# spool-labs/tape

Hardware: AMD Instinct MI355X
Metric: device-resident encode GiB/s, batched 4 MiB objects, 1 MI355X; % HBM peak (higher is better)
Workload: dtype u8; 1 GPU; Slicer::encode of 1024 x 4194304 B objects per GPU, Clay(20,7,16) rotated, 1 MB stripes; objects_per_gpu=1024, object_bytes=4194304, parallelism=objects partitioned over 1 GPU(s)

## Files before the change

### tape_amd/csrc/encode_dma.hip

```cpp
#include <atomic>
#include <string.h>
#include "kernels.hpp"
#include "gf_dev.hpp"
#include "dev_io.hpp"
#include "enc_common.hpp"

namespace tec {
namespace dma {

using enc::kQ;
using enc::pft3;
constexpr int K = 7;
constexpr int G = 6;
constexpr uint32_t RB = 90;
constexpr uint32_t RW = RB * 16;
constexpr uint32_t kOwnBlk = 7 * RB;
constexpr uint32_t kPartBlk = 9 * RB;
constexpr uint32_t kPartBase = kOwnBlk * 16;
constexpr uint32_t kSlotBytes = (kOwnBlk + kPartBlk) * 16;
constexpr uint32_t kRing = 2;
constexpr uint32_t kStageBase = kRing * kSlotBytes;
constexpr uint32_t kStageRows = 24;
constexpr uint32_t kMailBase = kStageBase + kStageRows * RW;
constexpr uint32_t kMailBytes = 64;
// ... 341 lines not shown
#if TEC_DMA_JX
        const uint32_t jx_base = (uint32_t)(reinterpret_cast<uintptr_t>(jdst) & 127u);
        const __amdgpu_buffer_rsrc_t rb_jx =
            __builtin_amdgcn_make_buffer_rsrc(jdst - jx_base, 0, (int)(dst_range + jx_base), 0x00020000);
#endif
        const uint32_t store_mask = J.store_mask;
        uint32_t sl_lane = lane + J.rot;
        sl_lane = (sl_lane >= 20u ? sl_lane - 20u : sl_lane) * slen;
        auto slice_off = [&](uint32_t node) -> uint32_t { return __builtin_amdgcn_readlane(sl_lane, node); };

        for (uint32_t z0 = z0b; z0 < z0e; z0++) {
            const bool lvl2 = z0 >= (uint32_t)K;
            const uint32_t type = lvl2 ? z0 - (K - 1) : 0u;
            for (uint32_t s = 0; s < (uint32_t)kQ; s++) {
                const uint32_t z = z0 * kQ + s;
                const uint32_t slot = (z & 1u) * kSlotBytes;
                const uint8_t *img = lds8 + slot + colw;
                auto out = [&](int r, uint32_t v) { st32(stg + r * RW, v); };
                uint32_t own[K], part[kQ];
#pragma unroll
                for (int x = 0; x < K; x++) own[x] = lds32(img + x * RW);
                if (z == ez && fixl) {
#pragma unroll
                    for (int x = 0; x < K; x++)
                        if ((uint32_t)x == ex) own[x] = fixw;
                    st32(lds8 + slot + ex * RW + colw, fixw);
                }
                uint32_t acc[20 - K];
                if (!lvl2) {
#pragma unroll
                    for (int x = 0; x < kQ; x++)
                        part[x] = lds32(img + kPartBase + x * RW - ((uint32_t)x > z0 ? RW : 0u));
                    if (z0 == ex && s == ez % kQ && fixl) {
#pragma unroll
                        for (int x = 0; x < kQ; x++)
                            if ((uint32_t)x == ez / kQ) part[x] = fixw;
                    }
                    uint32_t u[K];
#pragma unroll
                    for (int x = 0; x < K; x++) u[x] = (uint32_t)x == z0 ? own[x] : pft3(own[x], part[x]);
                    enc::mds7_slp<true>(u, acc);
#pragma unroll
                    for (int r = 0; r < 3; r++)
                        out(kRowC0 + r, acc[r] ^ mulc(kPft.t_p[1], part[K + r]));
                } else {
#pragma unroll
                    for (int x = 0; x < 9; x++) part[x] = lds32(img + kPartBase + x * RW);
                    uint32_t u[K];
#pragma unroll
                    for (int x = 0; x < K; x++) u[x] = pft3(own[x], part[x]);
                    enc::mds7_slp<false>(u, acc);
                    const uint32_t i0 = z0 - K;
#pragma unroll
                    for (int r = 0; r < 3; r++) {
                        if (r < 2) {
                            const uint32_t us = part[K + r], up = acc[r];
                            const uint32_t tt = xt(us ^ up);
                            out(kRowX + r, us ^ tt);
                            out(kRowC0 + r, (uint32_t)r < i0 ? up ^ tt : up);
                        } else {
                            out(kRowC0 + r, acc[r]);
                        }
                    }
                }
                switch (s) {
                    case 0: col1<0>(acc + 3, sl, out); break;
                    case 1: col1<1>(acc + 3, sl, out); break;
                    case 2: col1<2>(acc + 3, sl, out); break;
                    case 3: col1<3>(acc + 3, sl, out); break;
                    case 4: col1<4>(acc + 3, sl, out); break;
                    case 5: col1<5>(acc + 3, sl, out); break;
                    case 6: col1<6>(acc + 3, sl, out); break;
                    case 7: col1<7>(acc + 3, sl, out); break;
                    case 8: col1<8>(acc + 3, sl, out); break;
                    default: col1<9>(acc + 3, sl, out); break;
                }
                lds_barrier();
                const FlushTab::W &F = kFlush.w[type][s][wv];
                const uint32_t n = F.n;
                u32x4 d0[kCap], d1[kCap];
                uint32_t dst[kCap];
#pragma unroll
                for (int q = 0; q < kCap; q++) {
                    if ((uint32_t)q < n) {
                        const uint32_t it = F.item[q];
                        const uint32_t src = it & 0xffu;
                        const uint8_t *row = (src & 0x80u) ? lds8 + slot + (src & 0x7fu) * RW : lds8 + kStageBase + src * RW;
                        d0[q] = *reinterpret_cast<const u32x4 *>(row + lo0);
                        d1[q] = *reinterpret_cast<const u32x4 *>(row + lo1);
                        const uint32_t node = (it >> 8) & 0xffu, tz0 = (it >> 16) & 0xffu, ts = it >> 24;
                        dst[q] = slice_off(node) + ((tz0 == 0xffu ? z0 : tz0) * kQ + (ts == 0xffu ? s : ts)) * sc;
                        if (!((store_mask >> node) & 1u)) dst[q] = kDrop;
                    }
                }
                asm volatile("s_waitcnt vmcnt(%0)" ::"n"(kStoreLag) : "memory");
                lds_barrier();
#pragma unroll
                for (int q = 0; q < kCap; q++) {
                    if ((uint32_t)q < n) {
#if TEC_DMA_JX
                        const uint32_t ab = jx_base + dst[q], first = (ab + 127u) & ~127u;
                        const uint32_t o0 = first + 16u * lane - jx_base, o1 = first + 16u * (64u + lane) - jx_base;
                        const uint32_t lim = ((ab + (uint32_t)sc + 127u) & ~127u) - jx_base;
                        __builtin_amdgcn_raw_buffer_store_b128(d0[q], rb_jx, (int)(dst[q] == kDrop ? kDrop : o0), 0, kStAux);
                        __builtin_amdgcn_raw_buffer_store_b128(d1[q], rb_jx, (int)(dst[q] == kDrop || o1 >= lim ? kDrop : o1), 0, kStAux);
#else
                        __builtin_amdgcn_raw_buffer_store_b128(d0[q], rb_dst, (int)vo0, (int)dst[q], kStAux);
                        __builtin_amdgcn_raw_buffer_store_b128(d1[q], rb_dst, (int)vo1, (int)dst[q], kStAux);
#endif
                    }
                }
            }
        }
        if (wv == 0 && z0e == (uint32_t)kQ) {
            const uint32_t it = kFlush.extra, src = it & 0xffu;
            const uint8_t *row = lds8 + kStageBase + src * RW;
            const u32x4 e0 = *reinterpret_cast<const u32x4 *>(row + lo0);
            const u32x4 e1 = *reinterpret_cast<const u32x4 *>(row + lo1);
            const uint32_t node = (it >> 8) & 0xffu, tz0 = (it >> 16) & 0xffu, ts = it >> 24;
            const uint32_t d = ((store_mask >> node) & 1u)
                                   ? slice_off(node) + ((tz0 == 0xffu ? kQ - 1u : tz0) * kQ + (ts == 0xffu ? kQ - 1u : ts)) * sc
                                   : kDrop;
            __builtin_amdgcn_raw_buffer_store_b128(e0, rb_dst, (int)vo0, (int)d, kStAux);
            __builtin_amdgcn_raw_buffer_store_b128(e1, rb_dst, (int)vo1, (int)d, kStAux);
        }
    }
}

}

bool encode_dma_supported(int n, int k, uint32_t sc) { return n == 20 && k == 7 && sc > 1280u && sc <= 1440u && sc % 2 == 0; }

static uint32_t enc_slots() {
    const char *e = tec_knob("TEC_ENC_GRID");
    if (e && strcmp(e, "cu") != 0) {
        const long v = atol(e);
        return v < 0 ? 0u : (uint32_t)v;
    }
    static std::atomic<uint32_t> cached[64];
    int dev = 0;
    if (hipGetDevice(&dev) != hipSuccess || dev < 0 || dev >= 64) dev = 0;
    uint32_t v = cached[dev].load(std::memory_order_relaxed);
    if (!v) {
        int cus = 0;
        if (hipDeviceGetAttribute(&cus, hipDeviceAttributeMultiprocessorCount, dev) != hipSuccess || cus <= 0) cus = 256;
        v = 2u * (uint32_t)cus;
        cached[dev].store(v, std::memory_order_relaxed);
    }
    return v;
}

uint32_t encode_dma_grid(const EncArgs &a) { return enc_grid(enc_task_count(a), enc_slots()); }

hipError_t launch_encode_dma(bool masked, const EncArgs &a0, hipStream_t s) {
    if (a0.njobs == 0) return hipSuccess;
    if (!encode_dma_supported((int)a0.n, 7, a0.sc) || a0.njobs > 0x7fffffffu) return hipErrorInvalidValue;
    const void *fn = masked ? reinterpret_cast<const void *>(dma::enc_dma_kernel<true>)
                            : reinterpret_cast<const void *>(dma::enc_dma_kernel<false>);
#ifndef TEC_DMA_LDS_PAD
#define TEC_DMA_LDS_PAD 0
#endif
    const size_t lds = dma::kLdsBytes + TEC_DMA_LDS_PAD;
    hipError_t e = ensure_dyn_lds(fn, lds);
    if (e != hipSuccess) return e;
    if (a0.z0_count) {
        const uint32_t lim = a0.z0_limit ? a0.z0_limit : 10u;
        if (a0.z0_split == 0 || lim > 10u || a0.z0_first + (a0.z0_split - 1u) * a0.z0_count >= lim) return hipErrorInvalidValue;
    }
    const uint64_t ntasks = enc_task_count(a0);
    if (ntasks > 0x7fffffffu) return hipErrorInvalidValue;
    EncArgs a = a0;
    a.ntasks = (uint32_t)ntasks;
    const uint32_t grid = a.queue ? encode_dma_grid(a) : a.ntasks;
    if (masked)
        hipLaunchKernelGGL(dma::enc_dma_kernel<true>, dim3(grid), dim3(dma::kWaves * 64), lds, s, a);
    else
        hipLaunchKernelGGL(dma::enc_dma_kernel<false>, dim3(grid), dim3(dma::kWaves * 64), lds, s, a);
    return hipGetLastError();
}

}
```

### tape_amd/csrc/engine.cpp

```cpp
#include <hip/hip_runtime.h>
#include <string.h>
#include <stdio.h>
#include <stdlib.h>
#include <deque>
#include <map>
#include <unordered_map>
#include <mutex>
#include <vector>
#include <algorithm>
#include <functional>
#include <thread>
#include <atomic>
#include <chrono>
#include <condition_variable>
#include "../../include/tape_ec.h"
#include "kernels.hpp"
#include "sha256.hpp"
#include <array>
#include "clay_host.hpp"
#include "rs16.hpp"
#include "host_hash.hpp"
#include "copy_pool.hpp"
#include "dec_class.hpp"

using namespace tec;

namespace {

constexpr size_t kStripeSizes[3] = {100000, 1000000, 10000000};

thread_local char g_last_error[256] = "";
const bool g_no_dma_encode = [] {
    const char *e = tec_knob("TEC_ENCODE_KERNEL");
    return e && strcmp(e, "stage") == 0;
}();

const uint32_t g_enc_split = [] {
    const char *e = tec_knob("TEC_ENC_SPLIT");
    return e ? (uint32_t)atoi(e) : 512u;
}();
const uint32_t g_enc_split_batch = [] {
    const char *e = tec_knob("TEC_ENC_SPLIT_BATCH");
    const int v = e ? atoi(e) : 0;
    return (uint32_t)(v < 0 ? 0 : v > 7 ? 7 : v);
}();
const uint32_t g_enc_small = [] {
    const char *e = tec_knob("TEC_ENC_SMALL");
    return e ? (uint32_t)atoi(e) : 0u;
}();

const bool g_no_fold_repair = [] {
    const char *e = tec_knob("TEC_REPAIR_KERNEL");
    return e && strcmp(e, "stage") == 0;
}();

int hip_status(hipError_t e) {
    if (e == hipSuccess) return TE_OK;
    snprintf(g_last_error, sizeof(g_last_error), "%s (%d)", hipGetErrorString(e), (int)e);
    if (e == hipErrorOutOfMemory) return TE_ERR_OUT_OF_MEMORY;
    if (e == hipErrorNoDevice || e == hipErrorInvalidDevice) return TE_ERR_NO_DEVICE;
    return TE_ERR_HIP;
}

#define TE_HIP(expr)                              \
    do {                                          \
        hipError_t e_ = (expr);                   \
        if (e_ != hipSuccess) return hip_status(e_); \
    } while (0)

int sync_sleep(hipStream_t s) {
    hipEvent_t e = nullptr;
    if (hipEventCreateWithFlags(&e, hipEventDisableTiming | hipEventBlockingSync) != hipSuccess)
        return hip_status(hipStreamSynchronize(s));
    hipError_t r = hipEventRecord(e, s);
    if (r == hipSuccess) r = hipEventSynchronize(e);
    (void)hipEventDestroy(e);
    return hip_status(r);
}

int g_device_count = -1;
std::mutex g_dev_mu;

int device_count() {
    std::lock_guard<std::mutex> lk(g_dev_mu);
    if (g_device_count < 0) {
        int n = 0;
        if (hipGetDeviceCount(&n) != hipSuccess) n = 0;
        g_device_count = n;
    }
    return g_device_count;
}

struct DeviceGuard {
    int prev = -1;
    hipError_t err = hipSuccess;
    explicit DeviceGuard(int dev) {
        if (hipGetDevice(&prev) != hipSuccess) prev = -1;
        if (prev != dev) err = hipSetDevice(dev);
    }
    ~DeviceGuard() {
        int cur = -1;
        if (prev >= 0 && hipGetDevice(&cur) == hipSuccess && cur != prev) (void)hipSetDevice(prev);
    }
};

static bool vmm_bufs() {
    static const bool v = [] {
        const char *s = tec_knob("TEC_VMM_BUFS");
        return s && s[0] == '1';
    }();
    return v;
}

struct ReaderEvents {
    struct E {
        hipStream_t s = nullptr;
        hipEvent_t ev = nullptr;
        bool pending = false;
    };
    static constexpr size_t kMax = 16;
    std::vector<E> v;
    bool any() const {
        for (const E &e : v)
            if (e.pending) return true;
        return false;
    }
    hipError_t record(hipStream_t s) {
        E *slot = nullptr;
        for (E &e : v)
            if (e.s == s) slot = &e;
        if (!slot) {
            if (v.size() >= kMax) {
                if (hipError_t r = sync(); r != hipSuccess) return r;
                slot = &v[0];
                slot->s = s;
            } else {
                E e;
                e.s = s;
                if (hipError_t r = hipEventCreateWithFlags(&e.ev, hipEventDisableTiming); r != hipSuccess) return r;
                v.push_back(e);
                slot = &v.back();
            }
        }
        hipError_t r = hipEventRecord(slot->ev, s);
        if (r == hipSuccess) slot->pending = true;
        return r;
    }
    hipError_t wait(hipStream_t s) const {
        for (const E &e : v)
            if (e.pending && e.s != s)
                if (hipError_t r = hipStreamWaitEvent(s, e.ev, 0); r != hipSuccess) return r;
        return hipSuccess;
    }
    hipError_t sync() {
        for (E &e : v)
            if (e.pending) {
                if (hipError_t r = hipEventSynchronize(e.ev); r != hipSuccess) return r;
                e.pending = false;
            }
        return hipSuccess;
    }
    void destroy() {
        for (E &e : v)
            if (e.ev) (void)hipEventDestroy(e.ev);
        v.clear();
    }
};

static tec::CopyPool &copy_pool(int device) {
    static std::mutex mu;
    static tec::CopyPool *pools[65] = {};
    const int slot = device < 0 || device >= 64 ? 64 : device;
    std::lock_guard<std::mutex> g(mu);
    if (!pools[slot]) pools[slot] = new tec::CopyPool(std::max(0, std::min(3, hh::default_threads() - 1)));
    return *pools[slot];
}

struct DevBuf {
    void *p = nullptr;
    size_t cap = 0;
    hipMemGenericAllocationHandle_t vh{};
    bool vmm = false;
    hipError_t free_() {
        if (!p) return hipSuccess;
        hipError_t e = hipSuccess;
        if (vmm) {
            (void)hipDeviceSynchronize();
            e = hipMemUnmap(p, cap);
            if (e == hipSuccess) e = hipMemRelease(vh);
            if (e == hipSuccess) e = hipMemAddressFree(p, cap);
        } else {
            e = hipFree(p);
        }
        p = nullptr;
        cap = 0;
        vmm = false;
        return e;
    }
// ... 572 lines not shown
int te_slice_metadata_from_slice(const uint8_t *slice, size_t len, te_slice_metadata *out) {
    if (!slice || !out || len < TE_META_SIZE) return TE_ERR_INVALID_LAYOUT;
    const uint8_t *p = slice + len - TE_META_SIZE;
    out->version = get_u64(p);
    out->blob_len = get_u64(p + 8);
    out->stripe_size = get_u64(p + 16);
    out->encoding = get_u64(p + 24);
    out->params = get_u64(p + 32);
    out->chunk_index = get_u64(p + 40);
    if (!valid_stripe(out->stripe_size)) return TE_ERR_INVALID_LAYOUT;
    return TE_OK;
}

int te_slicer_geometry(const te_clay *c, size_t blob_len, te_geometry *g) {
    if (!c || !g) return TE_ERR_INVALID_ARG;
    const size_t S = te_pick_stripe_size(blob_len);
    const size_t ns = te_num_stripes(blob_len, S);
    const size_t eff = blob_len == 0 ? S : std::min(blob_len, S);
    const size_t cs = c->h.chunk_size_for(eff);
    g->stripe_size = S;
    g->num_stripes = ns;
    g->chunk_size = cs;
    g->sub_chunk_size = cs / (size_t)c->h.alpha;
    g->slice_len = ns * cs + TE_META_SIZE;
    return TE_OK;
}

}

namespace {

struct GeomKey {
    uint64_t cs, slice_len;
    bool masked;
    bool odd;
    bool operator<(const GeomKey &o) const {
        if (cs != o.cs) return cs < o.cs;
        if (slice_len != o.slice_len) return slice_len < o.slice_len;
        if (odd != o.odd) return odd < o.odd;
        return masked < o.masked;
    }
};

int ensure_stream(te_clay *c) {
    if (device_count() <= 0) return TE_ERR_NO_DEVICE;
    if (!c->stream) TE_HIP(hipStreamCreateWithFlags(&c->stream, hipStreamNonBlocking));
    return TE_OK;
}

using StripeSel = std::function<uint32_t(size_t, size_t)>;

int encode_enqueue(te_clay *c, const te_slicer_cfg *cfg, const uint8_t *d_data, const te_object *objs,
                   size_t nobj, uint8_t *d_out, hipStream_t s, bool raw, Arena *arena = nullptr,
                   const StripeSel &keep = StripeSel(), bool per_call = false) {
    const ClayHost &h = c->h;
    const int n = h.n;
    const int rotated = cfg ? cfg->rotated : 0;
    std::map<GeomKey, std::vector<EncJob>> groups;
    std::vector<MetaJob> metas;

    for (size_t i = 0; i < nobj; i++) {
        const te_object &o = objs[i];
        size_t S, ns, cs, slice_len;
        if (raw) {
            if (o.blob_len == 0) return TE_ERR_EMPTY_INPUT;
            cs = h.chunk_size_for(o.blob_len);
            S = cs * h.k;
            ns = 1;
            slice_len = cs;
        } else {
            te_geometry g;
            te_slicer_geometry(c, o.blob_len, &g);
            S = g.stripe_size; ns = g.num_stripes; cs = g.chunk_size; slice_len = g.slice_len;
        }
        if (cs % (size_t)h.alpha || slice_len > 0xffffffffull || cs > 0xffffffffull) return TE_ERR_TOO_MUCH_DATA;
        for (size_t st = 0; st < ns; st++) {
            const uint32_t store = keep ? keep(i, st) : ~0u;
            if (!store) continue;
            EncJob j{};
            j.store_mask = store;
            const uint64_t start = (uint64_t)st * S;
            j.src = d_data + o.data_off + start;
            j.src_len = o.blob_len == 0 ? 0 : std::min<uint64_t>(S, o.blob_len - start);
            j.dst = d_out + o.out_off + st * cs;
            j.rot = rotated ? (uint32_t)((st * TE_ROTATION_STEP) % n) : 0u;
            j.dst_skew = (uint32_t)(st * cs);
            const bool masked = ((reinterpret_cast<uintptr_t>(j.src) & 3u) + j.src_len) % 4 != 0;
            const bool odd = (reinterpret_cast<uintptr_t>(j.src) & 1u) != 0;
            groups[GeomKey{cs, slice_len, masked, odd}].push_back(j);
        }
        if (!raw && !keep) {
            MetaJob m{};
            m.dst = d_out + o.out_off + ns * cs;
            m.slice_len = slice_len;
            m.words[0] = 0;
            m.words[1] = o.blob_len;
            m.words[2] = S;
            m.words[3] = cfg ? cfg->encoding : TE_ENCODING_CLAY;
            m.words[4] = cfg ? cfg->params : TE_CLAY_DEFAULT_PARAMS;
            m.words[5] = o.chunk_index;
            metas.push_back(m);
        }
    }
    Arena &A = arena ? *arena : c->enc;
    A.img.clear();
    struct Launch { GeomKey key; size_t off, count; };
    std::vector<Launch> launches;
    for (auto &kv : groups) launches.push_back({kv.first, A.put(kv.second.data(), kv.second.size() * sizeof(EncJob)), kv.second.size()});
    const size_t meta_off = A.put(metas.data(), metas.size() * sizeof(MetaJob));
    size_t pat_off = 0, pool_off = 0;
    GpePattern pat{};
    std::vector<uint16_t> pool;
    std::vector<GpeJob> gjobs;
    std::vector<size_t> gjob_off;
    {
        uint64_t mask = 0;
        for (int i = h.k + h.nu; i < h.qt; i++) mask |= 1ull << i;
        if (!h.gpe_pattern(mask, pat, pool)) return TE_ERR_UNSUPPORTED;
        pat_off = A.put(&pat, sizeof(pat));
        pool_off = A.put(pool.data(), pool.size() * sizeof(uint16_t));
        for (auto &kv : groups) {
            std::vector<GpeJob> gj;
            for (const EncJob &e : kv.second) {
                GpeJob g{};
                g.in = e.src; g.out = e.dst; g.in_len = e.src_len; g.out_len = ~0ull; g.rot = e.rot; g.pattern = 0;
                gj.push_back(g);
            }
            gjob_off.push_back(A.put(gj.data(), gj.size() * sizeof(GpeJob)));
        }
    }
    int r = A.upload(s);
    if (r) return r;
    auto fast_path = [&](const Launch &L) {
        return c->fast_encode && !L.key.odd && (uint64_t)n * L.key.slice_len < 0x7fffffffull;
    };
    size_t total_stripes = 0;
    for (const Launch &L : launches) total_stripes += L.count;
    const bool small = per_call && !keep && total_stripes <= g_enc_small;
    auto dma_path = [&](const Launch &L) {
        return fast_path(L) && encode_dma_supported(n, h.k, (uint32_t)(L.key.cs / h.alpha)) && !g_no_dma_encode &&
               !small;
    };
    size_t scratch_bytes = 0;
    for (const Launch &L : launches) {
        if (!fast_path(L) || dma_path(L)) continue;
        const uint32_t wps = ((uint32_t)(L.key.cs / h.alpha) + 3) / 4;
        EncArgs a{};
        a.njobs = (uint32_t)L.count;
        a.groups_per_stripe = (wps + 63) / 64;
        a.groups_per_wg = small ? 1u : 0u;
        scratch_bytes = std::max(scratch_bytes, encode_rows_scratch_bytes(a));
    }
    const bool split_call = (per_call && total_stripes <= g_enc_split) || g_enc_split_batch;
    uint32_t nqueues = 0;
    for (const Launch &L : launches)
        if (dma_path(L)) nqueues += split_call ? 2u : 1u;
    const size_t queue_off = (scratch_bytes + 255) & ~(size_t)255;
    uint8_t *scratch = nullptr;
    if (scratch_bytes || nqueues) {
        r = A.workspace(queue_off + (size_t)nqueues * 4u, s, &scratch);
        if (r) return r;
    }
    uint32_t *const queues = reinterpret_cast<uint32_t *>(scratch + queue_off);
    uint32_t qi = 0;
    KTimer kt(s);
    if (!metas.empty())
        TE_HIP(launch_meta(A.at<MetaJob>(meta_off), (uint32_t)metas.size(), (uint32_t)n, s, queues, nqueues));
    else if (nqueues)
        TE_HIP(hipMemsetAsync(queues, 0, (size_t)nqueues * 4u, s));
    auto gpe_args = [&](size_t gi, const Launch &L, uint32_t word_base, uint32_t word_end) {
        const uint32_t cs = (uint32_t)L.key.cs, sc = cs / (uint32_t)h.alpha;
        (void)sc;
        GpeArgs a{};
        a.jobs = A.at<GpeJob>(gjob_off[gi]);
        a.patterns = A.at<GpePattern>(pat_off);
        a.plane_pool = A.at<uint16_t>(pool_off);
        a.njobs = (uint32_t)L.count;
        a.word_base = word_base;
        a.word_end = word_end;
        a.groups_per_stripe = (word_end - word_base + kGpeWords - 1) / kGpeWords;
        a.cs = cs; a.sc = cs / (uint32_t)h.alpha; a.q = h.q; a.t = h.t; a.k = h.k; a.nu = h.nu; a.n = n;
        a.alpha = h.alpha;
        a.in_stride = cs; a.out_stride = L.key.slice_len;
        a.in_rotated = 0; a.out_rotated = 1;
        a.out_mask = 0;
        for (int i = 0; i < h.qt; i++)
            if (h.int_to_ext(i) >= 0) a.out_mask |= 1ull << i;
        for (int i = 0; i < 16; i++) a.qpow[i] = h.qpow[i];
        return a;
    };
    size_t gi = 0;
    std::vector<std::pair<bool, EncArgs>> level2;
    te_encode_launch_stats &els = c->els;
    for (const Launch &L : launches) {
        const uint32_t cs = (uint32_t)L.key.cs, sc = cs / (uint32_t)h.alpha;
        const uint32_t wps = (sc + 3) / 4;
        const uint32_t full = sc / 4;
        if (dma_path(L)) {
            EncArgs a{};
            a.jobs = A.at<EncJob>(L.off);
            a.njobs = (uint32_t)L.count;
            a.cs = cs;
            a.sc = sc;
            a.slice_len = (uint32_t)L.key.slice_len;
            a.n = (uint32_t)n;
            a.queue = queues + qi++;
            if (split_call) {
                const uint32_t per = per_call ? 1u : g_enc_split_batch;
                a.z0_first = 0; a.z0_count = per; a.z0_split = (7 + per - 1) / per; a.z0_limit = 7;
                TE_HIP(launch_encode_dma(L.key.masked, a, s));
                els.dma_level1_launches++;
                a.z0_limit = 0;
                a.z0_first = 7; a.z0_count = 3; a.z0_split = 1;
                a.queue = queues + qi++;
                level2.push_back({L.key.masked, a});
            } else {
                TE_HIP(launch_encode_dma(L.key.masked, a, s));
            }
            els.dma_launches++;
            els.dma_stripes += L.count;
        } else if (fast_path(L)) {
            (void)full;
            EncArgs a{};
            a.jobs = A.at<EncJob>(L.off);
            a.njobs = (uint32_t)L.count;
            a.groups_per_stripe = (wps + 63) / 64;
            a.groups_per_wg = small ? 1u : 0u;
            a.words_per_stripe = wps;
            a.cs = cs;
            a.sc = sc;
            a.slice_len = (uint32_t)L.key.slice_len;
            a.n = (uint32_t)n;
            a.scratch = scratch;
            TE_HIP(launch_encode_rows(h.k, L.key.masked, a, s));
            els.stage_launches++;
            els.stage_masked_launches += L.key.masked ? 1u : 0u;
            els.stage_stripes += L.count;
            els.stage_g = encode_stage_g(a);
            els.stage_wgs = encode_stage_wgs(a);
        } else {
            TE_HIP(launch_gpe(gpe_args(gi, L, 0, wps), (uint32_t)pat.nerased, s));
            els.generic_launches++;
            els.generic_stripes += L.count;
        }
        gi++;
    }
    for (const auto &l2 : level2) {
        TE_HIP(launch_encode_dma(l2.first, l2.second, s));
        els.dma_launches++;
        els.dma_level2_launches++;
    }
    kt.stop();
    return A.mark_done(s);
}

}

namespace {

struct DecItem {
    uint64_t in_base;
    uint64_t slice_len, blob_len, stripe, ns, cs, out_off;
    uint32_t avail;
    int32_t lost = -1;
};

int decode_validate(const te_clay *c, const uint8_t *meta48, uint64_t slice_len, uint32_t avail, DecItem &it) {
    const ClayHost &h = c->h;
    const int na = __builtin_popcount(avail & ((h.n >= 32) ? 0xffffffffu : ((1u << h.n) - 1u)));
    if (na == 0) return TE_ERR_NOT_ENOUGH_SLICES;
    te_slice_metadata m;
    int r = te_slice_metadata_from_slice(meta48, TE_META_SIZE, &m);
    if (r) return r;
    const uint32_t pk = (uint32_t)((m.params >> 8) & 0xFF);
    if ((uint32_t)na < pk) return TE_ERR_NOT_ENOUGH_SLICES;
    it.blob_len = m.blob_len;
    it.stripe = m.stripe_size;
    it.slice_len = slice_len;
    it.avail = avail;
    if (m.blob_len == 0) { it.ns = 0; it.cs = 0; return TE_OK; }
    it.ns = (m.blob_len + m.stripe_size - 1) / m.stripe_size;
    const uint64_t total = slice_len >= TE_META_SIZE ? slice_len - TE_META_SIZE : 0;
    if (total == 0 || total % it.ns) return TE_ERR_INVALID_LAYOUT;
    it.cs = total / it.ns;
    if (na < h.k) return TE_ERR_NOT_ENOUGH_SLICES;
    if (it.cs % (uint64_t)h.alpha) return TE_ERR_BAD_ENCODING;
    const uint64_t last_take = m.blob_len - (it.ns - 1) * m.stripe_size;
    if (std::max<uint64_t>(it.ns > 1 ? m.stripe_size : 0, last_take) > it.cs * (uint64_t)h.k) return TE_ERR_INVALID_LAYOUT;
    return TE_OK;
}

bool compile_pattern(const ClayHost &h, uint64_t emask, int out_node, te_clay::DecCache &d) {
    const int n = h.n;
    if (!h.gpe_pattern(emask, d.P, d.planes)) return false;
    d.P.planes_off = 0;
    if (out_node >= 0 && dec_class_of(h, d.P) >= 0) dec_class_lost_first(d.P, out_node);
    if (decode_stage_k(h.k) && d.P.nknown == (uint32_t)h.k && d.P.nerased == (uint32_t)(n - h.k)) {
        DecProgHdr best{};
        std::vector<DecStep> best_steps;
        bool found = false;
        auto cost = [](const DecProgHdr &x) {
            return (decode_stage_rows(x.nslots, x.max_out) > 53 ? 1u << 20 : 0u) + x.nscratch;
        };
        static const int force = [] {
            const char *e = tec_knob("TEC_DEC_ORIENT");
            return e ? atoi(e) : -1;
        }();
        for (int orient = 0; orient < 2; orient++) {
            if (force >= 0 && orient != force) continue;
            DecProgHdr H;
            std::vector<DecStep> st;
            if (!h.dec_prog(d.P, orient, H, st, out_node) || !decode_stage_fits(H.nslots, H.max_out)) continue;
            if (!found || cost(H) < cost(best)) { best = H; best_steps.swap(st); found = true; d.orient = orient; }
        }
        bool ok = found;
        for (const DecStep &S : best_steps) {
            d.steps.emplace_back();
            ok = ok && ClayHost::dec_pack(S, d.steps.back());
        }
        d.steps.resize(d.steps.size() + 2);
        d.staged = ok && d.steps.size() == te_clay::DecStore::kSteps;
        d.H = best;
    }
    return true;
}

inline uint64_t dec_key(uint64_t emask, int out_node) { return emask | (uint64_t)(out_node + 1) << 48; }

const te_clay::DecCache *dec_pattern(te_clay *c, uint64_t emask, int out_node = -1) {
    const uint64_t key = dec_key(emask, out_node);
    auto f = c->dec_cache.find(key);
    if (f != c->dec_cache.end()) return &f->second;
    te_clay::DecCache d;
    if (!compile_pattern(c->h, emask, out_node, d)) return nullptr;
    return &c->dec_cache.emplace(key, std::move(d)).first->second;
}

void dec_precompile(te_clay *c, const std::vector<std::pair<uint64_t, int>> &keys) {
    std::vector<std::pair<uint64_t, int>> todo;
    for (const auto &k : keys)
        if (!c->dec_cache.count(dec_key(k.first, k.second))) todo.push_back(k);
    if (todo.size() < 8) return;
    std::vector<te_clay::DecCache> out(todo.size());
    std::vector<char> ok(todo.size(), 0);
    const unsigned hw = std::max(1u, std::thread::hardware_concurrency());
    const size_t nth = std::min<size_t>({16, (size_t)hw, (todo.size() + 7) / 8});
    std::atomic<size_t> next{0};
    auto work = [&] {
        for (size_t i; (i = next.fetch_add(1)) < todo.size();)
            ok[i] = compile_pattern(c->h, todo[i].first, todo[i].second, out[i]);
    };
    std::vector<std::thread> th;
    for (size_t t = 1; t < nth; t++) th.emplace_back(work);
    work();
    for (auto &t : th) t.join();
    for (size_t i = 0; i < todo.size(); i++)
        if (ok[i]) c->dec_cache.emplace(dec_key(todo[i].first, todo[i].second), std::move(out[i]));
}

struct StoreFill {
    uint32_t n0 = 0;
    bool wait_used = false;
    std::vector<GpePattern> pats;
    std::vector<DecProgHdr> hdrs;
// ... 3209 lines not shown
```

### tape_amd/csrc/kernels.hpp

```cpp
#pragma once
#include <hip/hip_runtime.h>
#include <stdint.h>
#include <stdlib.h>
#include "gf.hpp"
#include "dec_fixed.hpp"

namespace tec {

inline const char *tec_knob(const char *name) {
    const char *on = getenv("TEC_DEBUG_KNOBS");
    if (!on || on[0] != '1' || on[1] != 0) return nullptr;
    return getenv(name);
}

hipError_t ensure_dyn_lds(const void *fn, size_t bytes);

struct EncJob {
    const uint8_t *src;
    uint8_t *dst;
    uint64_t src_len;
    uint32_t rot;
    uint32_t dst_skew;
    uint32_t store_mask;
    uint32_t pad_;
};

struct EncArgs {
    const EncJob *jobs;
    uint32_t njobs;
    uint32_t groups_per_stripe;
    uint32_t words_per_stripe;
    uint32_t groups_per_wg;
    uint32_t wgs_per_stripe;
    uint32_t stripes_per_wg;
    uint32_t cs;
    uint32_t sc;
    uint32_t slice_len;
    uint32_t n;
    uint8_t *scratch;
    uint32_t z0_first, z0_count, z0_split;
    uint32_t z0_limit;
    uint32_t *queue;
    uint32_t ntasks;
};

struct EncTask {
    uint32_t job, z0b, z0e;
};
__host__ __device__ inline uint32_t enc_xcd_tile(uint32_t b, uint32_t nb) {
    const uint32_t full = nb & ~7u;
    if (b >= full) return b;
    return (b & 7u) * (full >> 3) + (b >> 3);
}
__host__ __device__ inline uint32_t enc_task_split(uint32_t z0_count, uint32_t z0_split) {
    return z0_count && z0_split ? z0_split : 1u;
}
__host__ __device__ inline EncTask enc_task(uint32_t t, uint32_t ntasks, uint32_t z0_first, uint32_t z0_count,
                                            uint32_t z0_split, uint32_t z0_limit) {
    const uint32_t tile = enc_xcd_tile(t, ntasks), split = enc_task_split(z0_count, z0_split);
    EncTask k;
    k.job = tile / split;
    const uint32_t part = tile - k.job * split;
    k.z0b = z0_count ? z0_first + part * z0_count : 0u;
    const uint32_t lim = z0_limit ? z0_limit : 10u, e = k.z0b + z0_count;
    k.z0e = z0_count ? (e < lim ? e : lim) : 10u;
    return k;
}
inline uint64_t enc_task_count(const EncArgs &a) { return (uint64_t)a.njobs * enc_task_split(a.z0_count, a.z0_split); }
inline uint32_t enc_grid(uint64_t ntasks, uint32_t slots) {
    return (uint32_t)(slots && slots < ntasks ? slots : ntasks);
}

struct MetaJob {
    uint8_t *dst;
    uint64_t slice_len;
    uint64_t words[6];
};

constexpr int kGpeMaxErased = 20;
constexpr int kGpeMaxKnown = 20;

struct GpePattern {
    uint64_t erased_mask;
    uint32_t nknown, nerased, nlevels, alpha;
    uint8_t known[kGpeMaxKnown];
    uint8_t erased[kGpeMaxErased];
    uint32_t level_start[16];
    uint32_t planes_off;
    uint32_t pad_;
    PermTab D[kGpeMaxErased][kGpeMaxKnown];
    uint32_t D4[13][7][4];
};
constexpr int kClsMaxE = 13, kClsMaxK = 7;

struct GpeJob {
    const uint8_t *in;
    uint8_t *out;
    uint64_t in_len;
    uint64_t out_len;
    uint32_t rot;
    uint32_t pattern;
};

struct GpeArgs {
    const GpeJob *jobs;
    const GpePattern *patterns;
    const uint16_t *plane_pool;
    uint32_t njobs;
    uint32_t word_base, word_end;
    uint32_t groups_per_stripe;
    uint32_t cs, sc, q, t, k, nu, n, alpha;
    uint64_t in_stride, out_stride;
    uint32_t in_rotated, out_rotated;
    uint64_t out_mask;
    uint32_t qpow[16];
};

struct RepPattern {
    uint64_t erased_mask, aloof_mask;
    uint32_t nknown, nerased, nlevels, beta;
    uint32_t lost;
    uint32_t pad_;
    uint8_t known[kGpeMaxKnown];
    uint8_t erased[kGpeMaxErased];
    uint32_t level_start[16];
    uint32_t planes_off;
    uint32_t pad2_;
    PermTab D[kGpeMaxErased][kGpeMaxKnown];
};

struct RepJob {
    const uint8_t *helper[kMaxNodes];
    uint8_t *out;
    uint32_t pattern;
    uint32_t aux;
};

constexpr int kRepQ = 10;
struct RepProg {
    uint32_t ekind[kGpeMaxErased];
    uint32_t erow[kGpeMaxErased];
    uint32_t enode[kGpeMaxErased];
    uint32_t knode0[kGpeMaxKnown];
    struct Step {
        uint32_t z, ri;
        uint32_t kkind[kGpeMaxKnown];
        uint32_t knode[kGpeMaxKnown];
        uint32_t krow[kGpeMaxKnown];
        uint32_t oplane[kRepQ];
    } step[kRepQ];
};

constexpr int kDecMaxK = 10, kDecMaxE = 13, kDecMaxOut = 16;
constexpr int kDecMaxOutProg = 32;
constexpr uint32_t kLocNone = 0xffffffffu;
enum : uint32_t { kLocStage = 0, kLocSlot = 1, kLocScratch = 2 };
enum : uint32_t { kKnRed = 0, kKnInput = 1, kKnLoc = 2, kKnPark = 3, kKnInputU = 4 };
enum : uint32_t { kErSkip = 0, kErRed = 1, kErType1 = 2, kErPark = 3, kErFinish = 4, kErType1U = 5 };
struct DecStep {
    uint32_t z;
    uint32_t nout;
    uint32_t out[kDecMaxOutProg];
    uint32_t kk[kDecMaxK];
    uint32_t kp[kDecMaxK];
    uint32_t kout[kDecMaxK];
    uint32_t kpark[kDecMaxK];
    uint32_t kpout[kDecMaxK];
    uint32_t ek[kDecMaxE];
    uint32_t ep[kDecMaxE];
    uint32_t ed0[kDecMaxE], ed1[kDecMaxE];
    uint32_t epd[kDecMaxE];
};
constexpr uint32_t kLoc10None = 0x3ffu;
enum : uint32_t { kDpHdr = 0, kDpKd = 1, kDpEd = kDpKd + kDecMaxK, kDpEo = kDpEd + kDecMaxE,
                  kDpOut = kDpEo + kDecMaxE, kDpWords = 48 };
struct DecStepP {
    uint32_t w[kDpWords];
};
static_assert(kDpOut + kDecMaxOut / 2 <= kDpWords, "packed step");
struct DecProgHdr {
    uint32_t nsteps, nslots, nscratch, max_out;
    uint32_t knode[kDecMaxK];
};

struct RepArgs {
    const RepJob *jobs;
    const RepPattern *patterns;
    const uint16_t *plane_pool;
    const uint16_t *plane_ind;
    uint32_t njobs, words_per_stripe, groups_per_stripe;
    uint32_t cs, sc, q, t, alpha;
    uint32_t qpow[16];
    uint32_t wgs_per_stripe;
    const RepProg *progs;
};

constexpr int kGpeWords = 4;
constexpr int kGpePlaneThreads = 32;

struct DecArgs {
    const GpeJob *jobs;
    const GpePattern *patterns;
    const DecProgHdr *hdrs;
    const DecStepP *steps;
    const uint32_t *step_off;
    uint8_t *scratch;
    uint32_t njobs, words_per_stripe, wgs_per_stripe;
    uint32_t cs, sc, n, nk, lds_rows, nscratch_max;
    uint64_t in_stride, out_stride;
    uint32_t gmax;
};
hipError_t launch_decode_stage(DecArgs a, hipStream_t s);
size_t decode_stage_scratch_bytes(const DecArgs &a);
uint32_t decode_stage_rows(uint32_t nslots, uint32_t max_out);
bool decode_stage_fits(uint32_t nslots, uint32_t max_out);
uint32_t decode_stage_g(uint32_t words_per_stripe, uint32_t gmax = 0);

using dfix_args = dfix::Args;
static_assert(sizeof(dfix::Job) == sizeof(GpeJob) && offsetof(dfix::Job, rot) == offsetof(GpeJob, rot), "dfix::Job");
struct DecJitKernel {
    hipFunction_t fn;
    size_t lds;
    uint32_t nscratch;
    uint32_t wb;
};
struct DecJit;
struct ClayHost;
DecJit *dec_jit_new(int device);
void dec_jit_free(DecJit *j);
void dec_jit_set(DecJit *j, int mode, uint64_t min_stripes);
void dec_jit_counts(DecJit *j, uint32_t timeout_ms, uint32_t *ready, uint32_t *pending, uint32_t *failed);
void dec_jit_hold(DecJit *j);
void dec_jit_unhold(DecJit *j);
const DecJitKernel *dec_jit_get(DecJit *j, const ClayHost &h, const GpePattern &P, int orient, int G, int wb, uint64_t stripes);
struct DecJitGeom { uint32_t wb, wps, G, wgs; };
DecJitGeom dec_jit_geom(uint32_t sc);
hipError_t launch_dec_fixed(const DecJitKernel &k, const dfix_args &a, uint32_t G, hipStream_t s);
bool decode_stage_k(int k);

bool dec_class_info(int id, uint32_t *nslots, uint32_t *nscratch);
uint32_t dec_class_wgs(uint32_t sc, uint32_t G);
size_t dec_class_scratch_bytes(int id, uint32_t njobs, uint32_t sc, uint32_t G);
hipError_t launch_dec_class(int id, const GpeJob *jobs, const GpePattern *patterns, uint32_t njobs, uint32_t sc,
                            uint64_t in_stride, uint64_t out_stride, uint32_t n, uint8_t *scratch, uint32_t G,
                            hipStream_t s);

constexpr int kCommitMaxLeaves = 64;
struct CommitArgs {
    const uint8_t *slices;
    uint64_t obj_stride, slice_len;
    uint32_t n, nobj, height;
    uint8_t *leaf;
    uint8_t *root;
    uint8_t *proof;
};
hipError_t launch_commit(const CommitArgs &a, hipStream_t s);

struct VerifyItem {
    uint64_t offset;
    uint64_t len;
    uint32_t expected;
    uint32_t object;
    uint32_t bit;
    uint32_t index;
};
struct VerifyArgs {
    const uint8_t *data;
    const VerifyItem *items;
    uint32_t nitems;
    const uint8_t *expected;
    uint8_t *digests;
    uint32_t *ok;
    uint32_t *good_mask;
};
constexpr uint64_t kVerifyBlocksPerLaunch = 1536;
__host__ __device__ inline uint64_t verify_blocks(uint64_t len) { return (len + 4u + 8u) / 64u + 1u; }
hipError_t launch_verify(const VerifyArgs &a, const VerifyItem *h_items, hipStream_t s);

hipError_t launch_encode_rows(int k, bool masked, const EncArgs &a, hipStream_t s);
uint32_t encode_stage_g(const EncArgs &a);
uint32_t encode_stage_wgs(const EncArgs &a);
bool encode_dma_supported(int n, int k, uint32_t sc);
hipError_t launch_encode_dma(bool masked, const EncArgs &a, hipStream_t s);
uint32_t encode_dma_grid(const EncArgs &a);
hipError_t launch_meta(const MetaJob *jobs, uint32_t njobs, uint32_t n, hipStream_t s, uint32_t *zero = nullptr,
                       uint32_t nzero = 0);
struct CopyJob {
    const uint8_t *src;
    uint8_t *dst;
    uint64_t len;
    uint64_t valid;
};
hipError_t launch_gather(const CopyJob *jobs, uint32_t njobs, hipStream_t s);
hipError_t launch_gpe(const GpeArgs &a, uint32_t max_erased, hipStream_t s);

constexpr uint32_t kRs16MaxK = 64;
struct Rs16EncArgs {
    const uint8_t *in;
    uint8_t *out;
    uint64_t in_stride, out_stride, seg_in, seg_out;
    const uint16_t *lut;
    uint32_t k, m, c, high, work_len, span, elems;
    uint32_t one_chunk;
};
constexpr uint32_t kRs16DecPtrs = 256;
struct Rs16DecArgs {
    const uint8_t *ptr[kRs16DecPtrs];
    const uint16_t *lut;
    uint32_t k, nmiss, elems;
};
constexpr uint32_t kRs16MatMaxG = 16;
constexpr uint32_t kRs16MatLds = 80 * 1024;
struct Rs16MatArgs {
    const uint8_t *in;
    uint8_t *out;
    uint64_t in_stride, out_stride, seg_in, seg_out;
    const uint8_t *ptr[kRs16DecPtrs];
    const uint16_t *tab;
    const uint32_t *ktab;
    uint32_t k, rows, elems, segments, ptrs;
    uint32_t rstride;
};
#ifndef TEC_RS16_MAT_TV
#define TEC_RS16_MAT_TV 0
#endif
inline bool rs16_mat_tailv(uint32_t rows) { return TEC_RS16_MAT_TV && rows % 8 == 1 && rows > 1; }
#ifndef TEC_RS16_MAT_NARROW
#define TEC_RS16_MAT_NARROW 1
#endif
inline uint32_t rs16_mat_tail_bytes(uint32_t rows) {
    const uint32_t G = (rows + 3) / 4;
    if (!(G & 1) || rs16_mat_tailv(rows)) return 0;
    const uint32_t t = rows - 8 * (G / 2);
    return !TEC_RS16_MAT_NARROW || t > 2 ? 8u : 2u * t;
}
inline uint32_t rs16_mat_block_bytes(uint32_t rows) { return ((rows + 3) / 4 / 2) * 256u + 16u * rs16_mat_tail_bytes(rows); }
inline size_t rs16_mat_bytes(uint32_t k, uint32_t rows) {
    return (size_t)k * 4u * rs16_mat_block_bytes(rows);
}
inline size_t rs16_mat_image_bytes(uint32_t k, uint32_t rows) {
    return rs16_mat_bytes(k, rows) + (rs16_mat_tailv(rows) ? (size_t)k * 64u : 0u);
}
inline bool rs16_mat_supported(uint32_t k, uint32_t rows) {
    return k >= 1 && k <= 32 && rows >= 1 && (rows + 3) / 4 <= kRs16MatMaxG && rs16_mat_bytes(k, rows) <= kRs16MatLds;
}
hipError_t launch_rs16_matrix(const Rs16MatArgs &a, hipStream_t s);
hipError_t launch_rs16_encode(const Rs16EncArgs &a, uint32_t segments, hipStream_t s);
hipError_t launch_rs16_decode(const Rs16DecArgs &a, uint32_t segments, hipStream_t s);
hipError_t launch_repair(const RepArgs &a, uint32_t max_erased, hipStream_t s);
hipError_t launch_repair_stage(RepArgs a, hipStream_t s);
int repair_fold_column(uint32_t q, uint32_t t, uint32_t k, uint32_t beta, uint32_t sc, uint32_t lost,
                       uint64_t erased_mask, uint64_t aloof_mask);
hipError_t launch_repair_fold(RepArgs a, hipStream_t s);
bool repair_stage_supported(uint32_t q, uint32_t beta, uint32_t sc, uint32_t nerased, uint32_t nknown, uint64_t aloof_mask);
uint32_t repair_fold_g(uint32_t words_per_stripe);
uint32_t repair_stage_g(uint32_t words_per_stripe);
inline uint32_t repair_wgs(uint32_t words_per_stripe, uint32_t g) { return ((words_per_stripe + 63) / 64 + g - 1) / g; }
bool encode_rows_supported(int n, int k, int d);
size_t encode_rows_scratch_bytes(const EncArgs &a);

}
```

Before: 808.1 GiB/s.

## Split tail jobs of batched DMA encode into finer z0 tasks to balance final wave

For large batches on the DMA encode path, the last `slots` jobs are broken into per-row level-1 tasks plus a separate level-2 launch, while head jobs stay whole-job tasks. The goal is to cut the tail imbalance of the persistent queue, where the last few whole-job tasks leave most CUs idle. The cost is an extra kernel launch and a queue, plus more complex task indexing in the kernel.

```diff
diff --git a/tape_amd/csrc/encode_dma.hip b/tape_amd/csrc/encode_dma.hip
--- a/tape_amd/csrc/encode_dma.hip
+++ b/tape_amd/csrc/encode_dma.hip
@@ -517,6 +517,12 @@
 
 uint32_t encode_dma_grid(const EncArgs &a) { return enc_grid(enc_task_count(a), enc_slots()); }
 
+uint32_t encode_dma_slots(bool *knob) {
+    const char *e = tec_knob("TEC_ENC_GRID");
+    if (knob) *knob = e && strcmp(e, "cu") != 0;
+    return enc_slots();
+}
+
 hipError_t launch_encode_dma(bool masked, const EncArgs &a0, hipStream_t s) {
     if (a0.njobs == 0) return hipSuccess;
     if (!encode_dma_supported((int)a0.n, 7, a0.sc) || a0.njobs > 0x7fffffffu) return hipErrorInvalidValue;
@@ -532,10 +538,16 @@
         const uint32_t lim = a0.z0_limit ? a0.z0_limit : 10u;
         if (a0.z0_split == 0 || lim > 10u || a0.z0_first + (a0.z0_split - 1u) * a0.z0_count >= lim) return hipErrorInvalidValue;
     }
+    if (a0.tail_jobs && (a0.tail_jobs > a0.njobs || !a0.z0_count || a0.z0_first || !a0.z0_limit || a0.z0_limit > 7u))
+        return hipErrorInvalidValue;
     const uint64_t ntasks = enc_task_count(a0);
     if (ntasks > 0x7fffffffu) return hipErrorInvalidValue;
     EncArgs a = a0;
     a.ntasks = (uint32_t)ntasks;
+    if (a.tail_jobs) {
+        a.z0_first = a.njobs - a.tail_jobs;
+        a.z0_limit |= kEncTailFlag;
+    }
     const uint32_t grid = a.queue ? encode_dma_grid(a) : a.ntasks;
     if (masked)
         hipLaunchKernelGGL(dma::enc_dma_kernel<true>, dim3(grid), dim3(dma::kWaves * 64), lds, s, a);
diff --git a/tape_amd/csrc/engine.cpp b/tape_amd/csrc/engine.cpp
--- a/tape_amd/csrc/engine.cpp
+++ b/tape_amd/csrc/engine.cpp
@@ -44,6 +44,19 @@
     const int v = e ? atoi(e) : 0;
     return (uint32_t)(v < 0 ? 0 : v > 7 ? 7 : v);
 }();
+constexpr uint32_t kEncTailDefault = ~0u;
+int64_t enc_tail_knob() {
+    const char *e = tec_knob("TEC_ENC_TAIL");
+    if (!e) return -1;
+    if (strcmp(e, "all") == 0) return 0xffffffffll;
+    const long long v = atoll(e);
+    return (int64_t)(v < 0 ? 0 : v > 0xffffffffll ? 0xffffffffll : v);
+}
+uint32_t enc_tail_rows() {
+    const char *e = tec_knob("TEC_ENC_TAIL_ROWS");
+    const int v = e ? atoi(e) : 1;
+    return (uint32_t)(v < 1 ? 1 : v > 7 ? 7 : v);
+}
 const uint32_t g_enc_small = [] {
     const char *e = tec_knob("TEC_ENC_SMALL");
     return e ? (uint32_t)atoi(e) : 0u;
@@ -922,9 +935,18 @@
         scratch_bytes = std::max(scratch_bytes, encode_rows_scratch_bytes(a));
     }
     const bool split_call = (per_call && total_stripes <= g_enc_split) || g_enc_split_batch;
+    const int64_t tail_knob = enc_tail_knob();
+    auto tail_of = [&](const Launch &L) -> uint32_t {
+        if (!dma_path(L) || split_call) return 0u;
+        if (tail_knob >= 0) return (uint32_t)std::min<uint64_t>((uint64_t)tail_knob, L.count);
+        bool knob = false;
+        const uint32_t slots = encode_dma_slots(&knob);
+        if (!kEncTailDefault || knob || !slots || L.count < 4ull * slots) return 0u;
+        return std::min(kEncTailDefault, slots);
+    };
     uint32_t nqueues = 0;
     for (const Launch &L : launches)
-        if (dma_path(L)) nqueues += split_call ? 2u : 1u;
+        if (dma_path(L)) nqueues += split_call || tail_of(L) ? 2u : 1u;
     const size_t queue_off = (scratch_bytes + 255) & ~(size_t)255;
     uint8_t *scratch = nullptr;
     if (scratch_bytes || nqueues) {
@@ -980,6 +1002,19 @@
                 a.z0_first = 0; a.z0_count = per; a.z0_split = (7 + per - 1) / per; a.z0_limit = 7;
                 TE_HIP(launch_encode_dma(L.key.masked, a, s));
                 els.dma_level1_launches++;
+                a.z0_limit = 0;
+                a.z0_first = 7; a.z0_count = 3; a.z0_split = 1;
+                a.queue = queues + qi++;
+                level2.push_back({L.key.masked, a});
+            } else if (const uint32_t tail = tail_of(L)) {
+                const uint32_t per = enc_tail_rows();
+                a.tail_jobs = tail;
+                a.z0_first = 0; a.z0_count = per; a.z0_split = (7 + per - 1) / per; a.z0_limit = 7;
+                TE_HIP(launch_encode_dma(L.key.masked, a, s));
+                els.dma_level1_launches++;
+                a.jobs += L.count - tail;
+                a.njobs = tail;
+                a.tail_jobs = 0;
                 a.z0_limit = 0;
                 a.z0_first = 7; a.z0_count = 3; a.z0_split = 1;
                 a.queue = queues + qi++;
diff --git a/tape_amd/csrc/kernels.hpp b/tape_amd/csrc/kernels.hpp
--- a/tape_amd/csrc/kernels.hpp
+++ b/tape_amd/csrc/kernels.hpp
@@ -42,6 +42,7 @@
     uint32_t z0_limit;
     uint32_t *queue;
     uint32_t ntasks;
+    uint32_t tail_jobs;
 };
 
 struct EncTask {
@@ -55,10 +56,27 @@
 __host__ __device__ inline uint32_t enc_task_split(uint32_t z0_count, uint32_t z0_split) {
     return z0_count && z0_split ? z0_split : 1u;
 }
+constexpr uint32_t kEncTailFlag = 0x80000000u;
 __host__ __device__ inline EncTask enc_task(uint32_t t, uint32_t ntasks, uint32_t z0_first, uint32_t z0_count,
                                             uint32_t z0_split, uint32_t z0_limit) {
+    EncTask k;
+    if (z0_limit & kEncTailFlag) {
+        const uint32_t head = z0_first;
+        if (t < head) {
+            k.job = enc_xcd_tile(t, head);
+            k.z0b = 0u;
+            k.z0e = 10u;
+            return k;
+        }
+        const uint32_t u = t - head, split = enc_task_split(z0_count, z0_split);
+        const uint32_t j = u / split, part = u - j * split;
+        k.job = head + j;
+        k.z0b = part * z0_count;
+        const uint32_t lim = z0_limit & ~kEncTailFlag, e = k.z0b + z0_count;
+        k.z0e = e < lim ? e : lim;
+        return k;
+    }
     const uint32_t tile = enc_xcd_tile(t, ntasks), split = enc_task_split(z0_count, z0_split);
-    EncTask k;
     k.job = tile / split;
     const uint32_t part = tile - k.job * split;
     k.z0b = z0_count ? z0_first + part * z0_count : 0u;
@@ -66,7 +84,17 @@
     k.z0e = z0_count ? (e < lim ? e : lim) : 10u;
     return k;
 }
-inline uint64_t enc_task_count(const EncArgs &a) { return (uint64_t)a.njobs * enc_task_split(a.z0_count, a.z0_split); }
+__host__ __device__ inline EncTask enc_task(uint32_t t, uint32_t ntasks, uint32_t njobs, uint32_t tail_jobs,
+                                            uint32_t z0_first, uint32_t z0_count, uint32_t z0_split,
+                                            uint32_t z0_limit) {
+    if (tail_jobs == 0) return enc_task(t, ntasks, z0_first, z0_count, z0_split, z0_limit);
+    return enc_task(t, ntasks, njobs - tail_jobs, z0_count, z0_split, z0_limit | kEncTailFlag);
+}
+inline uint64_t enc_task_count(const EncArgs &a) {
+    const uint64_t split = enc_task_split(a.z0_count, a.z0_split);
+    if (a.tail_jobs) return (uint64_t)(a.njobs - a.tail_jobs) + (uint64_t)a.tail_jobs * split;
+    return (uint64_t)a.njobs * split;
+}
 inline uint32_t enc_grid(uint64_t ntasks, uint32_t slots) {
     return (uint32_t)(slots && slots < ntasks ? slots : ntasks);
 }
@@ -283,6 +311,7 @@
 bool encode_dma_supported(int n, int k, uint32_t sc);
 hipError_t launch_encode_dma(bool masked, const EncArgs &a, hipStream_t s);
 uint32_t encode_dma_grid(const EncArgs &a);
+uint32_t encode_dma_slots(bool *knob);
 hipError_t launch_meta(const MetaJob *jobs, uint32_t njobs, uint32_t n, hipStream_t s, uint32_t *zero = nullptr,
                        uint32_t nzero = 0);
 struct CopyJob {
```

Result: slower. 776.4 GiB/s (-3.9%).
